# CityU-AIM-Group/MultiModal-learning

Measured on AMD Instinct MI355X. Metric: ROI-tiles/sec (teacher+student distill step), higher is better.
Workload: dtype bf16; 1 GPU; BASELINE configs[1]: teacher+student distill step, bf16, batch 64 per GPU, 512x512 tiles, 320-d omic, CRD P=300/K=700->P2=20/K2=512, n_data=1024, GK-Refine on, Adam+EMA, dropout 0.1; tiles_per_gpu=64, tile=512, global_batch=64, parallelism=single, launch=one captured HIP graph per step, input_pipeline=inputs resident in HBM when the timed region starts

## Files before the change

### multimodal-learning_amd/csrc/conv_wgrad.hip

```cpp
#include "ph_common.h"
#include "ph_kernels.h"
#include "tap_common.h"

namespace {

__device__ __forceinline__ int sw_piece(int pix, int piece) { return piece ^ (((pix >> 1) & 1) << 1); }

template <typename T, int S, int TH, int KS>
struct WgCfg {
  static constexpr bool SPLIT = is_f32<T>::value;
  static constexpr bool HPM = is_hp<T>::value;
  static constexpr int TW = 16, BM = TH * TW;
  static constexpr int HPH = (TH - 1) * S + KS, HPW = (TW - 1) * S + KS, HP = HPH * HPW;
  static constexpr int HPP = (HP + 7) / 8 * 8;
  static constexpr int D_BYTES = BM * 128, X_BYTES = HPP * 128;
  static constexpr int NP = SPLIT ? PH_NPLANES : 1;
  static constexpr int LDS_BYTES = SPLIT ? (D_BYTES + X_BYTES) * NP : 2 * (D_BYTES + X_BYTES);
  static constexpr int NT = KS * KS;
};

template <typename T>
__device__ __forceinline__ void stage_row(const T* src, bool ok, unsigned char* base, int plane_bytes, int off) {
  if constexpr (!is_f32<T>::value) {
    u32x4 v = {0u, 0u, 0u, 0u};
    if (ok) v = *reinterpret_cast<const u32x4*>(src);
    *reinterpret_cast<u32x4*>(base + off) = v;
  } else {
    float v[8];
#pragma unroll
    for (int q = 0; q < 8; ++q) v[q] = 0.f;
    if (ok) load8(src, v);
    bf16x8 p0, p1, p2;
#pragma unroll
    for (int q = 0; q < 8; ++q) { bf16 a, b, c; split3_bf16(v[q], a, b, c); p0[q] = a; p1[q] = b; p2[q] = c; }
    *reinterpret_cast<bf16x8*>(base + off) = p0;
    *reinterpret_cast<bf16x8*>(base + plane_bytes + off) = p1;
    *reinterpret_cast<bf16x8*>(base + 2 * plane_bytes + off) = p2;
  }
}

__device__ __forceinline__ bf16x8 tr_pair(const unsigned char* base, int off0, int off1) {
  typedef __attribute__((address_space(3))) s16x4 lds_s16x4;
  s16x4 a = __builtin_amdgcn_ds_read_tr16_b64_v4i16((lds_s16x4*)(base + off0));
  s16x4 b = __builtin_amdgcn_ds_read_tr16_b64_v4i16((lds_s16x4*)(base + off1));
  union { s16x4 s[2]; bf16x8 v; } u;
  u.s[0] = a; u.s[1] = b;
  return u.v;
}

template <typename T, int S, int TH, int KS>
__global__ __launch_bounds__(256) void wgrad_kernel(PhWgrad p) {
  using C = WgCfg<T, S, TH, KS>;
  constexpr bool SPLIT = C::SPLIT, HPM = C::HPM;
  constexpr int TW = C::TW, BM = C::BM, HPW = C::HPW, HP = C::HP, NT = C::NT, NP = C::NP;
  typedef typename std::conditional<HPM, f16, T>::type TI;
  constexpr int EW = HPM ? 2 : 1;
  extern __shared__ __attribute__((aligned(16))) unsigned char smem[];
  unsigned char* ldsD = smem;
  unsigned char* ldsX = smem + C::D_BYTES * NP;

  const int tid = threadIdx.x, lane = tid & 63;
  const int wave = __builtin_amdgcn_readfirstlane(tid >> 6);
  const int cf = wave >> 1, kf = wave & 1;
  const int cin_blocks = p.Cin >> 6;
  const int co0 = (blockIdx.x / cin_blocks) << 6, ci0 = (blockIdx.x % cin_blocks) << 6;
  const int chunk = blockIdx.y;
  const int tiles_w = (p.OW + TW - 1) / TW, tiles_h = (p.OH + TH - 1) / TH;
  const int tiles_img = tiles_w * tiles_h, ntiles = tiles_img * p.B;
  const int t_begin = chunk * p.tiles_per_chunk;
  const int t_end = min(ntiles, t_begin + p.tiles_per_chunk);
  const TI* X = reinterpret_cast<const TI*>(p.x);
  const TI* DY = reinterpret_cast<const TI*>(p.dy);
  const long xpix = (p.x_pix_stride ? p.x_pix_stride : p.Cin) * EW;
  const long xrow = (p.x_row_stride ? p.x_row_stride : (long)p.IW * p.Cin) * EW;
  const long ximg = (p.x_img_stride ? p.x_img_stride : (long)p.IH * p.IW * p.Cin) * EW;
  const long dpix = (long)p.Cout * EW;

  f32x16 acc[NT];
#pragma unroll
  for (int t = 0; t < NT; ++t)
#pragma unroll
    for (int q = 0; q < 16; ++q) acc[t][q] = 0.f;

  const int q4 = (lane & 15) >> 2, p4 = lane & 3, colhalf = (lane >> 4) & 1, khalf = lane >> 5;
  const int pieceA = cf * 2 + colhalf, pieceB = kf * 2 + colhalf;

  auto compute = [&](const unsigned char* dD, const unsigned char* dX) {
#pragma unroll 2
    for (int kk = 0; kk < BM / 16; ++kk) {
      const int t0 = kk * 16 + 8 * khalf + q4, t1 = t0 + 4;
      const int offA0 = t0 * 128 + sw_piece(t0, pieceA) * 32 + p4 * 8;
      const int offA1 = t1 * 128 + sw_piece(t1, pieceA) * 32 + p4 * 8;
      bf16x8 a[NP];
#ifdef PH_ABL_WG_NOLDS
#pragma unroll
      for (int pl = 0; pl < NP; ++pl) { bf16x8 z; asm volatile("" : "=v"(z)); a[pl] = z; }
#else
#pragma unroll
      for (int pl = 0; pl < NP; ++pl)
        if (pl < 2 || p.prod6) a[pl] = tr_pair(dD + pl * C::D_BYTES, offA0, offA1);
#endif
      const int hb0 = ((t0 >> 4) * S) * HPW + (t0 & 15) * S;
      const int hb1 = ((t1 >> 4) * S) * HPW + (t1 & 15) * S;
#pragma unroll
      for (int t = 0; t < NT; ++t) {
        const int toff = (t / KS) * HPW + (t % KS);
        const int h0 = hb0 + toff, h1 = hb1 + toff;
        const int offB0 = h0 * 128 + sw_piece(h0, pieceB) * 32 + p4 * 8;
        const int offB1 = h1 * 128 + sw_piece(h1, pieceB) * 32 + p4 * 8;
        bf16x8 bq[NP];
#ifdef PH_ABL_WG_NOLDS
#pragma unroll
        for (int pl = 0; pl < NP; ++pl) { bf16x8 z; asm volatile("" : "=v"(z) : "v"(offB0 + offB1)); bq[pl] = z; }
#else
#pragma unroll
        for (int pl = 0; pl < NP; ++pl)
          if (pl < 2 || p.prod6) bq[pl] = tr_pair(dX + pl * C::X_BYTES, offB0, offB1);
#endif
        if constexpr (SPLIT) {
#define PH_MM(PI, PJ) acc[t] = __builtin_amdgcn_mfma_f32_32x32x16_bf16(a[PI], bq[PJ], acc[t], 0, 0, 0);
          if (p.prod6) { PH_SPLIT_PAIRS_LO(PH_MM) }
          PH_SPLIT_PAIRS_HI(PH_MM)
#undef PH_MM
        } else if constexpr (HPM) {
          acc[t] = __builtin_amdgcn_mfma_f32_32x32x16_f16(__builtin_bit_cast(f16x8, a[0]), __builtin_bit_cast(f16x8, bq[0]), acc[t], 0, 0, 0);
        } else {
          acc[t] = __builtin_amdgcn_mfma_f32_32x32x16_bf16(a[0], bq[0], acc[t], 0, 0, 0);
        }
      }
    }
  };

  constexpr bool PIPE = !SPLIT && S == 1 && KS == 3 && (BM / 16 == TH);
  constexpr int PBUF = C::D_BYTES + C::X_BYTES;
  const int u_lane = 8 * khalf + q4;
  const int baseA = u_lane * 128 + ((pieceA ^ (((u_lane >> 1) & 1) << 1)) << 5) + p4 * 8;
  const int baseB = u_lane * 128 + (pieceB << 5) + p4 * 8;
  const int bE0 = baseB ^ (((u_lane >> 1) & 1) << 6), bE1 = bE0 ^ 64;
  const int bO0 = baseB ^ ((((u_lane >> 1) ^ u_lane) & 1) << 6), bO1 = bO0 ^ 64;
  if constexpr (PIPE) {
#pragma unroll
    for (int t = 0; t < NT; ++t) asm volatile("" : "+a"(acc[t]));
  }
  auto compute_p = [&](const int boff) __attribute__((always_inline)) {
    if constexpr (PIPE) {
      const unsigned char* dD = smem + boff;
      const unsigned char* dX = dD + C::D_BYTES;
      constexpr int NI = (BM / 16) * 9, LA = 3;
      bf16x8 af[2], bfr[4];
      auto ldA = [&](const int kk) { return tr_pair(dD, baseA + kk * 2048, baseA + 512 + kk * 2048); };
      auto ldB = [&](const int i) {
        const int kk = i / 9, t = i % 9;
        const int toff = (t / 3) * HPW + (t % 3);
        const int flip = ((kk & 1) ^ ((toff >> 1) & 1)) & 1;
        const int base = (toff & 1) ? (flip ? bO1 : bO0) : (flip ? bE1 : bE0);
        const int imm = (kk * HPW + toff) * 128;
        return tr_pair(dX, base + imm, base + imm + 512);
      };
      af[0] = ldA(0);
#pragma unroll
      for (int i = 0; i < LA; ++i) bfr[i] = ldB(i);
#pragma unroll
      for (int i = 0; i < NI; ++i) {
        const int kk = i / 9, t = i % 9;
        if (i + LA < NI) bfr[(i + LA) & 3] = ldB(i + LA);
        if (t == 4 && kk + 1 < BM / 16) af[(kk + 1) & 1] = ldA(kk + 1);
        if constexpr (HPM) asm volatile("v_mfma_f32_32x32x16_f16 %0, %1, %2, %0" : "+a"(acc[t]) : "v"(af[kk & 1]), "v"(bfr[i & 3]));
        else asm volatile("v_mfma_f32_32x32x16_bf16 %0, %1, %2, %0" : "+a"(acc[t]) : "v"(af[kk & 1]), "v"(bfr[i & 3]));
        __builtin_amdgcn_sched_barrier(0);
      }
    }
  };

  if constexpr (SPLIT) {
    for (int tt = t_begin; tt < t_end; ++tt) {
      const int b = tt / tiles_img, ti = tt - b * tiles_img;
      const int r0 = (ti / tiles_w) * TH, c0 = (ti % tiles_w) * TW;
      __syncthreads();
      for (int i = tid; i < BM * 8; i += 256) {
        const int pix = i >> 3, ch = i & 7;
        const int r = r0 + (pix >> 4), c = c0 + (pix & 15);
        const bool ok = r < p.OH && c < p.OW;
        const int off = pix * 128 + sw_piece(pix, ch >> 1) * 32 + (ch & 1) * 16;
        stage_row<T>(DY + (((size_t)b * p.OH + r) * p.OW + c) * p.Cout + co0 + ch * 8, ok, ldsD, C::D_BYTES, off);
      }
      const int iy_base = r0 * S - p.pad, ix_base = c0 * S - p.pad;
      for (int i = tid; i < HP * 8; i += 256) {
        const int pix = i >> 3, ch = i & 7;
        const int hr = pix / HPW, hc = pix - hr * HPW;
        const int iy = iy_base + hr, ix = ix_base + hc;
        const bool ok = iy >= 0 && iy < p.IH && ix >= 0 && ix < p.IW;
        const int off = pix * 128 + sw_piece(pix, ch >> 1) * 32 + (ch & 1) * 16;
        stage_row<T>(X + (size_t)b * ximg + (size_t)iy * xrow + (size_t)ix * xpix + ci0 + ch * 8, ok, ldsX, C::X_BYTES, off);
      }
      __syncthreads();
      compute(ldsD, ldsX);
    }
  } else {
    const unsigned lds0 = (unsigned)(size_t)(lds_uchar*)smem;
    constexpr int BUF = C::D_BYTES + C::X_BYTES;
    const unsigned char* zero = reinterpret_cast<const unsigned char*>(p.zeros);
    const int nt = t_end > t_begin ? t_end - t_begin : 0;
    const bool hi1 = HPM && p.hp_hi_only;
    const int nitems = (HPM && !hi1) ? 3 * nt : nt;
    const int dblk = HPM ? (co0 >> 6) * 128 : co0, xblk = HPM ? (ci0 >> 6) * 128 : ci0;
    auto issue = [&](int item, int buf) {
      int pass = 0, tt = t_begin + item;
      if constexpr (HPM) { if (!hi1) { pass = item / nt; tt = t_begin + (item - pass * nt); } else pass = 2; }
      const int dpl = (HPM && pass == 1) ? 64 : 0, xpl = (HPM && pass == 0) ? 64 : 0;
      const int b = tt / tiles_img, ti = tt - b * tiles_img;
      const int r0 = (ti / tiles_w) * TH, c0 = (ti % tiles_w) * TW;
      unsigned char* dD = smem + buf * BUF;
      unsigned char* dX = dD + C::D_BYTES;
      for (int i0 = wave * 64; i0 < BM * 8; i0 += 256) {
        const int i = i0 + lane, pix = i >> 3, pos = i & 7;
        const int ch = sw_piece(pix, pos >> 1) * 2 + (pos & 1);
        const int r = r0 + (pix >> 4), c = c0 + (pix & 15);
        const bool ok = r < p.OH && c < p.OW;
        const void* src = ok ? (const void*)(DY + (((size_t)b * p.OH + r) * p.OW + c) * dpix + dblk + dpl + ch * 8)
                             : (const void*)zero;
        lds_dma16(src, __builtin_amdgcn_readfirstlane(lds0 + (unsigned)(dD - smem) + i0 * 16));
      }
      const int iy_base = r0 * S - p.pad, ix_base = c0 * S - p.pad;
      for (int i0 = wave * 64; i0 < C::HPP * 8; i0 += 256) {
        const int i = i0 + lane, pix = i >> 3, pos = i & 7;
        const int ch = sw_piece(pix, pos >> 1) * 2 + (pos & 1);
        const int hr = pix / HPW, hc = pix - hr * HPW;
        const int iy = iy_base + hr, ix = ix_base + hc;
        const bool ok = pix < HP && iy >= 0 && iy < p.IH && ix >= 0 && ix < p.IW;
        const void* src = ok ? (const void*)(X + (size_t)b * ximg + (size_t)iy * xrow + (size_t)ix * xpix + xblk + xpl + ch * 8)
                             : (const void*)zero;
        lds_dma16(src, __builtin_amdgcn_readfirstlane(lds0 + (unsigned)(dX - smem) + i0 * 16));
      }
    };
    if (nitems > 0) issue(0, 0);
    asm volatile("s_waitcnt vmcnt(0)" ::: "memory");
    __syncthreads();
    int buf = 0;
    for (int it = 0; it < nitems; ++it) {
#ifndef PH_ABL_WG_NODMA
      if (it + 1 < nitems) issue(it + 1, buf ^ 1);
#endif
      if constexpr (HPM) {
        if (!hi1 && it == 2 * nt) {
#pragma unroll
          for (int t = 0; t < NT; ++t)
#pragma unroll
            for (int q = 0; q < 16; ++q) {
              if constexpr (PIPE) {
                float tmp_;
                asm volatile("v_accvgpr_read_b32 %1, %0\n\ts_nop 4\n\tv_mul_f32 %1, %2, %1\n\ts_nop 4\n\tv_accvgpr_write_b32 %0, %1\n\ts_nop 4"
                             : "+a"(acc[t][q]), "=&v"(tmp_) : "v"(PH_HP_LO_INV));
              } else {
                acc[t][q] *= PH_HP_LO_INV;
              }
            }
        }
      }
      if constexpr (PIPE) compute_p(buf * PBUF);
      else compute(smem + buf * BUF, smem + buf * BUF + C::D_BYTES);
      asm volatile("s_waitcnt vmcnt(0)" ::: "memory");
      __syncthreads();
      buf ^= 1;
    }
  }
  float* slab = p.slab + (size_t)chunk * NT * p.Cout * p.Cin;
#pragma unroll
  for (int t = 0; t < NT; ++t)
#pragma unroll
    for (int q = 0; q < 16; ++q) {
      const int row = co0 + cf * 32 + (q & 3) + 8 * (q >> 2) + 4 * khalf;
      const int col = ci0 + kf * 32 + (lane & 31);
#ifdef PH_ABL_WG_NOSLAB
      asm volatile("" ::"v"(acc[t][q]), "v"(row + col));
#else
      if constexpr (PIPE) {
        float* dst = slab + ((size_t)t * p.Cout + row) * p.Cin + col;
        asm volatile("global_store_dword %0, %1, off" : : "v"(dst), "a"(acc[t][q]) : "memory");
      } else {
        slab[((size_t)t * p.Cout + row) * p.Cin + col] = acc[t][q];
      }
#endif
      if (PIPE && q == 15) __builtin_amdgcn_sched_barrier(0);
    }
}

template <typename T, int S, int TH, int KS>
int launch_wg(const PhWgrad& p, hipStream_t st) {
  using C = WgCfg<T, S, TH, KS>;
  auto kern = wgrad_kernel<T, S, TH, KS>;
  static bool attr_done = false;
  if (!attr_done) {
    if (hipFuncSetAttribute(reinterpret_cast<const void*>(kern), hipFuncAttributeMaxDynamicSharedMemorySize,
                            C::LDS_BYTES) != hipSuccess)
      return PH_ELAUNCH;
    attr_done = true;
  }
  dim3 grid((p.Cout / 64) * (p.Cin / 64), p.nchunks);
  void* tok = nullptr;
  if (ph_prof_on())
    ph_prof_begin2(PH_CLS_WGRAD, 2.0 * p.B * p.OH * p.OW * (double)p.Cout * p.KS * p.KS * p.Cin,
                   ((double)p.B * p.IH * p.IW * p.Cin + (double)p.B * p.OH * p.OW * p.Cout) * sizeof(T) +
                       (double)p.nchunks * p.KS * p.KS * p.Cout * p.Cin * 4.0, st, &tok);
  hipLaunchKernelGGL(kern, grid, dim3(256), C::LDS_BYTES, st, p);
  ph_prof_end(tok, st);
  PH_LAUNCH_CHECK();
  return PH_OK;
}

template <typename T>
int launch_wg_T(const PhWgrad& p, hipStream_t st) {
  if (p.S == 1 && p.KS == 3) return launch_wg<T, 1, 8, 3>(p, st);
  if (p.S == 2 && p.KS == 3) return launch_wg<T, 2, 4, 3>(p, st);
  if (p.S == 2 && p.KS == 1) return launch_wg<T, 2, 4, 1>(p, st);
  if (p.S == 1 && p.KS == 1) return launch_wg<T, 1, 8, 1>(p, st);
  return PH_EINVAL;
}

__global__ __launch_bounds__(256) void wgrad_reduce_kernel(const float* __restrict__ slab, float* __restrict__ dw,
                                                           int nchunks, int NT, int Cout, int Cin,
                                                           const float* __restrict__ unscale) {
  const size_t n = (size_t)NT * Cout * Cin;
  const int e = threadIdx.x & 63, cl = threadIdx.x >> 6;
  const size_t i = (size_t)blockIdx.x * 64 + e;
  float s0 = 0.f, s1 = 0.f, s2 = 0.f, s3 = 0.f;
  if (i < n) {
    int c = cl;
    for (; c + 12 < nchunks; c += 16) {
      s0 += slab[(size_t)c * n + i];
      s1 += slab[(size_t)(c + 4) * n + i];
      s2 += slab[(size_t)(c + 8) * n + i];
      s3 += slab[(size_t)(c + 12) * n + i];
    }
    for (; c < nchunks; c += 4) s0 += slab[(size_t)c * n + i];
  }
  __shared__ float sh[4][64];
  sh[cl][e] = (s0 + s1) + (s2 + s3);
  __syncthreads();
  if (cl == 0 && i < n) {
    float s = (sh[0][e] + sh[1][e]) + (sh[2][e] + sh[3][e]);
    if (unscale) s *= unscale[1];
    const int ci = i % Cin;
    const int co = (i / Cin) % Cout;
    const int t = i / ((size_t)Cin * Cout);
    dw[((size_t)co * Cin + ci) * NT + t] = s;
  }
}

__global__ void pack_w_kernel(const float* __restrict__ w, bf16* __restrict__ planes, int O, int I, int NT,
                              int dgrad) {
  const size_t n = (size_t)NT * O * I;
  const size_t i = (size_t)blockIdx.x * blockDim.x + threadIdx.x;
  if (i >= n) return;
  int t, o, ii;
  if (!dgrad) { ii = i % I; o = (i / I) % O; t = i / ((size_t)I * O); }
  else        { o = i % O; ii = (i / O) % I; t = i / ((size_t)I * O); }
  const float v = w[((size_t)o * I + ii) * NT + t];
  bf16 a, b, c;
  split3_bf16(v, a, b, c);
  planes[i] = a; planes[n + i] = b; planes[2 * n + i] = c;
}

__global__ void pack_w_stem_kernel(const float* __restrict__ w, bf16* __restrict__ planes) {
  const int i = blockIdx.x * blockDim.x + threadIdx.x;
  if (i >= 7 * 64 * 32) return;
  const int k = i & 31, co = (i >> 5) & 63, kh = i >> 11;
  const int kw = k >> 2, ch = k & 3;
  float v = 0.f;
  if (kw < 7 && ch < 3) v = w[((co * 3 + ch) * 7 + kh) * 7 + kw];
  bf16 a, b, c;
  split3_bf16(v, a, b, c);
  planes[i] = a; planes[7 * 64 * 32 + i] = b; planes[2 * 7 * 64 * 32 + i] = c;
}

__global__ void pack_all_kernel(PhPackAll t, bf16* __restrict__ packed, int nplanes) {
  const size_t i = (size_t)blockIdx.x * blockDim.x + threadIdx.x;
  if (i >= t.total) return;
  int u = 0;
#pragma unroll 1
  while (u + 1 < t.n && i >= t.start[u + 1]) ++u;
  const size_t e = i - t.start[u];
  const int O = t.O[u], I = t.I[u], NT = t.NT[u];
  const size_t n = (size_t)NT * O * I;
  const int ii = e % I, o = (e / I) % O, tp = e / ((size_t)I * O);
  const float v = t.w[u][((size_t)o * I + ii) * NT + tp];
  bf16 a, b, c;
  split3_bf16(v, a, b, c);
  const size_t fdst = t.dst_fwd[u] + e;
  const size_t ddst = t.dst_dg[u] + ((size_t)tp * I + ii) * O + o;
  packed[fdst] = a; packed[ddst] = a;
  if (nplanes == 3) {
    packed[fdst + n] = b; packed[fdst + 2 * n] = c;
    packed[ddst + n] = b; packed[ddst + 2 * n] = c;
  }
}

struct PackTiles { int tstart[21]; };
__device__ __forceinline__ size_t frag64_index(int r, int k) {
  return (size_t)(((k >> 5) * 4 + (r & 3)) * 512 + ((((k >> 3) & 3) << 4) + (r >> 2)) * 8 + (k & 7));
}
template <int NP>
__global__ __launch_bounds__(256) void pack_all_tiled_kernel(PhPackAll t, PackTiles pt, bf16* __restrict__ packed) {
  __shared__ bf16 sh[NP][32][32 * 9 + 2];
  int u = 0;
#pragma unroll 1
  while (u + 1 < t.n && (int)blockIdx.x >= pt.tstart[u + 1]) ++u;
  const int O = t.O[u], I = t.I[u], NT = t.NT[u];
  const int tile = (int)blockIdx.x - pt.tstart[u];
  const int itiles = I >> 5;
  const int o0 = (tile / itiles) << 5, i0 = (tile % itiles) << 5;
  const size_t n = (size_t)NT * O * I;
  const int run = 32 * NT;
  for (int idx = threadIdx.x; idx < 32 * run; idx += 256) {
    const int o = idx / run, r = idx - o * run;
    const float v = t.w[u][((size_t)(o0 + o) * I + i0) * NT + r];
    if constexpr (NP == 1) {
      sh[0][o][r] = (bf16)v;
    } else {
      bf16 a, b, c;
      split3_bf16(v, a, b, c);
      sh[0][o][r] = a; sh[1][o][r] = b; sh[2][o][r] = c;
    }
  }
  __syncthreads();
  for (int idx = threadIdx.x; idx < 32 * run; idx += 256) {
    const int x = idx & 31, y = (idx >> 5) & 31, tp = idx >> 10;
    const size_t fdst = t.dst_fwd[u] + ((size_t)tp * O + o0 + y) * I + i0 + x;
    const size_t ddst = t.dst_dg[u] + ((size_t)tp * I + i0 + y) * O + o0 + x;
#pragma unroll
    for (int pl = 0; pl < NP; ++pl) {
      packed[fdst + pl * n] = sh[pl][y][x * NT + tp];
      packed[ddst + pl * n] = sh[pl][x][y * NT + tp];
    }
    if constexpr (NP == 1) {
      if (NT == 9 && O == 2 * I) {
        const int o = o0 + y, i = i0 + x;
        packed[t.dst_fwd[u] + n + (size_t)tp * O * I + (size_t)((o >> 6) * (I >> 6) + (i >> 6)) * 4096 + frag64_index(o & 63, i & 63)] = sh[0][y][x * NT + tp];
      }
      if (NT == 9 && O == I && I >= 128) {
        const int o = o0 + y, i = i0 + x;
        packed[t.dst_fwd[u] + n + (size_t)tp * O * I + (size_t)((o >> 6) * (I >> 6) + (i >> 6)) * 4096 + frag64_index(o & 63, i & 63)] = sh[0][y][x * NT + tp];
        const int r = i0 + y, k = o0 + x;
        packed[t.dst_dg[u] + n + (size_t)tp * I * O + (size_t)((r >> 6) * (O >> 6) + (k >> 6)) * 4096 + frag64_index(r & 63, k & 63)] = sh[0][x][y * NT + tp];
      }
    }
  }
}

__device__ __forceinline__ size_t hp_k(int k) { return (size_t)(k >> 6) * 192 + (k & 63); }
__device__ __forceinline__ void hp_w3(float v, f16& b0, f16& b1, f16& b2) {
  hp_split(v, b2, b1);
  b0 = (f16)((float)b2 * PH_HP_LO);
}
__device__ __forceinline__ size_t ph5_frag_index(int r, int k) { return frag64_index(r, k); }
template <bool ONE>
__global__ __launch_bounds__(256) void pack_all_tiled_hp_kernel(PhPackAll t, PackTiles pt, f16* __restrict__ packed, int dgrad_only) {
  __shared__ float sh[32][32 * 9 + 1];
  int u = 0;
#pragma unroll 1
  while (u + 1 < t.n && (int)blockIdx.x >= pt.tstart[u + 1]) ++u;
  const int O = t.O[u], I = t.I[u], NT = t.NT[u];
  const int ffwd = t.frag[u] & 3, fdg = (t.frag[u] >> 2) & 3;
  const int tile = (int)blockIdx.x - pt.tstart[u];
  const int itiles = I >> 5;
  const int o0 = (tile / itiles) << 5, i0 = (tile % itiles) << 5;
  const int run = 32 * NT;
  for (int idx = threadIdx.x; idx < 32 * run; idx += 256) {
    const int o = idx / run, r = idx - o * run;
    sh[o][r] = t.w[u][((size_t)(o0 + o) * I + i0) * NT + r];
  }
  __syncthreads();
  for (int idx = threadIdx.x; idx < 32 * run; idx += 256) {
    const int x = idx & 31, y = (idx >> 5) & 31, tp = idx >> 10;
    f16 b0, b1, b2;
    if (!ONE || dgrad_only == 0) {
      hp_w3(sh[y][x * NT + tp], b0, b1, b2);
      if (ffwd == PH_WFRAG_TAP5) {
        f16* d = packed + t.dst_fwd[u] + (size_t)tp * 12288 + ph5_frag_index(o0 + y, i0 + x);
        d[0] = b0; d[4096] = b1; d[8192] = b2;
      } else if (ffwd == PH_WFRAG_TAP6) {
        const int o = o0 + y, i = i0 + x;
        f16* d = packed + t.dst_fwd[u] + (size_t)tp * O * 3 * I + (size_t)(((o >> 6) * (I >> 6) + (i >> 6)) * 3) * 4096 + ph5_frag_index(o & 63, i & 63);
        d[0] = b0; d[4096] = b1; d[8192] = b2;
      } else {
        f16* d = packed + t.dst_fwd[u] + ((size_t)tp * O + o0 + y) * (3 * (size_t)I) + hp_k(i0 + x);
        d[0] = b0; d[64] = b1; d[128] = b2;
      }
    }
    if (!ONE || dgrad_only == 1) {
      hp_w3(sh[x][y * NT + tp], b0, b1, b2);
      if (fdg == PH_WFRAG_TAP5) {
        f16* d = packed + t.dst_dg[u] + (size_t)tp * 12288 + ph5_frag_index(i0 + y, o0 + x);
        d[0] = b0; d[4096] = b1; d[8192] = b2;
      } else {
        f16* d = packed + t.dst_dg[u] + ((size_t)tp * I + i0 + y) * (3 * (size_t)O) + hp_k(o0 + x);
        d[0] = b0; d[64] = b1; d[128] = b2;
      }
    }
  }
}

__global__ void pack_w_stem_hp_kernel(const float* __restrict__ w, f16* __restrict__ packed) {
  const int i = blockIdx.x * blockDim.x + threadIdx.x;
  if (i >= 7 * 64 * 32) return;
  const int k = i & 31, co = (i >> 5) & 63, kh = i >> 11;
  const int kw = k >> 2, ch = k & 3;
  float v = 0.f;
  if (kw < 7 && ch < 3) v = w[((co * 3 + ch) * 7 + kh) * 7 + kw];
  f16 b0, b1, b2;
  hp_w3(v, b0, b1, b2);
  packed[i] = b0; packed[7 * 64 * 32 + i] = b1; packed[2 * 7 * 64 * 32 + i] = b2;
}

}

int ph_pack_w_stem_hp_launch(const float* w, void* packed, hipStream_t st) {
  hipLaunchKernelGGL(pack_w_stem_hp_kernel, dim3((7 * 64 * 32 + 255) / 256), dim3(256), 0, st, w, (f16*)packed);
  PH_LAUNCH_CHECK();
  return PH_OK;
}

int ph_pack_w_hp_launch(const float* w, void* packed, int O, int I, int KS, int dgrad, int wfrag, hipStream_t st) {
  if ((O & 31) || (I & 31) || (KS != 1 && KS != 3)) return PH_EINVAL;
  if (wfrag == PH_WFRAG_TAP5 && !(O == 64 && I == 64 && KS == 3)) return PH_EINVAL;
  if (wfrag == PH_WFRAG_TAP6 && !(O == 2 * I && KS == 3 && !dgrad)) return PH_EINVAL;
  if (wfrag < 0 || wfrag > PH_WFRAG_TAP6) return PH_EINVAL;
  PhPackAll t{};
  t.n = 1; t.w[0] = w; t.O[0] = O; t.I[0] = I; t.NT[0] = KS * KS; t.dst_fwd[0] = 0; t.dst_dg[0] = 0;
  t.frag[0] = dgrad ? wfrag << 2 : wfrag;
  t.start[0] = 0; t.start[1] = t.total = (size_t)KS * KS * O * I;
  PackTiles pt;
  pt.tstart[0] = 0; pt.tstart[1] = (O >> 5) * (I >> 5);
  hipLaunchKernelGGL(pack_all_tiled_hp_kernel<true>, dim3(pt.tstart[1]), dim3(256), 0, st, t, pt, (f16*)packed, dgrad ? 1 : 0);
  PH_LAUNCH_CHECK();
  return PH_OK;
}

int ph_pack_all_launch(const PhPackAll* t, void* packed, int nplanes, hipStream_t st) {
  bool tiled = t->n <= 20;
  PackTiles pt;
  pt.tstart[0] = 0;
  for (int u = 0; u < t->n && tiled; ++u) {
    if ((t->O[u] & 31) || (t->I[u] & 31) || t->NT[u] > 9) tiled = false;
    pt.tstart[u + 1] = pt.tstart[u] + (t->O[u] >> 5) * (t->I[u] >> 5);
  }
  if (nplanes == -3) {
    if (!tiled) return PH_EINVAL;
    for (int u = 0; u < t->n; ++u) {
      const int ff = t->frag[u] & 3, fd = (t->frag[u] >> 2) & 3;
      if ((ff == PH_WFRAG_TAP5 || fd == PH_WFRAG_TAP5) && !(t->O[u] == 64 && t->I[u] == 64 && t->NT[u] == 9)) return PH_EINVAL;
      if (ff == PH_WFRAG_TAP6 && !(t->O[u] == 2 * t->I[u] && t->NT[u] == 9)) return PH_EINVAL;
      if (ff == 3 || fd == 3 || fd == PH_WFRAG_TAP6) return PH_EINVAL;
    }
    hipLaunchKernelGGL(pack_all_tiled_hp_kernel<false>, dim3(pt.tstart[t->n]), dim3(256), 0, st, *t, pt, (f16*)packed, 0);
  } else if (tiled && nplanes == 1)
    hipLaunchKernelGGL(pack_all_tiled_kernel<1>, dim3(pt.tstart[t->n]), dim3(256), 0, st, *t, pt, (bf16*)packed);
  else if (tiled && nplanes == 3)
    hipLaunchKernelGGL(pack_all_tiled_kernel<3>, dim3(pt.tstart[t->n]), dim3(256), 0, st, *t, pt, (bf16*)packed);
  else
    hipLaunchKernelGGL(pack_all_kernel, dim3((unsigned)((t->total + 255) / 256)), dim3(256), 0, st, *t, (bf16*)packed,
                       nplanes);
  PH_LAUNCH_CHECK();
  return PH_OK;
}

int ph_wgrad_tile_h(int S) { return S == 1 ? 8 : 4; }

int ph_wgrad_launch(const PhWgrad* p, int prec, hipStream_t st) {
  if (p->Cin % 64 || p->Cout % 64 || p->nchunks < 1) return PH_EINVAL;
  if (prec == PH_PREC_BF16) { ph_dispatch_note(PH_DK_WGRAD_BF16); return launch_wg_T<bf16>(*p, st); }
  if (prec == PH_PREC_FP16X3 || prec == PH_PREC_FP16X1) {
    PhWgrad q = *p;
    q.hp_hi_only = prec == PH_PREC_FP16X1;
    ph_dispatch_note(PH_DK_WGRAD_HP16);
    return launch_wg_T<hp16>(q, st);
  }
  if (PH_IS_SPLIT_PREC(prec)) {
    PhWgrad q = *p;
    q.prod6 = prec == PH_PREC_BF16X6;
    ph_dispatch_note(PH_DK_WGRAD_F32);
    return launch_wg_T<float>(q, st);
  }
  return PH_EINVAL;
}

int ph_wgrad_reduce_launch(const float* slab, float* dw, int nchunks, int KS, int Cout, int Cin, const float* unscale,
                           hipStream_t st) {
  const size_t n = (size_t)KS * KS * Cout * Cin;
  hipLaunchKernelGGL(wgrad_reduce_kernel, dim3((unsigned)((n + 63) / 64)), dim3(256), 0, st, slab, dw, nchunks,
                     KS * KS, Cout, Cin, unscale);
  PH_LAUNCH_CHECK();
  return PH_OK;
}

int ph_pack_w_fwd_launch(const float* w, void* planes, int O, int I, int KS, hipStream_t st) {
  const size_t n = (size_t)KS * KS * O * I;
  hipLaunchKernelGGL(pack_w_kernel, dim3((unsigned)((n + 255) / 256)), dim3(256), 0, st, w, (bf16*)planes, O, I,
                     KS * KS, 0);
  PH_LAUNCH_CHECK();
  return PH_OK;
}
int ph_pack_w_dgrad_launch(const float* w, void* planes, int O, int I, int KS, hipStream_t st) {
  const size_t n = (size_t)KS * KS * O * I;
  hipLaunchKernelGGL(pack_w_kernel, dim3((unsigned)((n + 255) / 256)), dim3(256), 0, st, w, (bf16*)planes, O, I,
                     KS * KS, 1);
  PH_LAUNCH_CHECK();
  return PH_OK;
}
int ph_pack_w_stem_launch(const float* w, void* planes, hipStream_t st) {
  hipLaunchKernelGGL(pack_w_stem_kernel, dim3((7 * 64 * 32 + 255) / 256), dim3(256), 0, st, w, (bf16*)planes);
  PH_LAUNCH_CHECK();
  return PH_OK;
}
```

Measured before the change: 6354 tiles/s.

## Add lean wgrad loop with precomputed DMA offsets and reordered MFMA reuse

Adds a LEAN variant of the weight-gradient kernel, gated by a PH_WG_LEAN switch. It precomputes per-lane LDS-DMA offsets and validity bitmasks once per block and walks tiles incrementally, instead of recomputing addresses and bounds for every item. Its compute loop reorders the MFMA stream so each staged halo row fragment serves all three kh taps. DMA issues for the next item are interleaved into the MFMA stream. The cost is more kernel variants and register state. Whether it runs depends on the switch default and on a 32-bit offset fit check.

Result: faster. 6479 tiles/s (median of 6 runs) (+2.0%).

```diff
diff --git a/multimodal-learning_amd/csrc/conv_wgrad.hip b/multimodal-learning_amd/csrc/conv_wgrad.hip
--- a/multimodal-learning_amd/csrc/conv_wgrad.hip
+++ b/multimodal-learning_amd/csrc/conv_wgrad.hip
@@ -1,6 +1,8 @@
 #include "ph_common.h"
 #include "ph_kernels.h"
 #include "tap_common.h"
+
+PH_SWITCH(wg_lean, "PH_WG_LEAN")
 
 namespace {
 
@@ -17,6 +19,7 @@
   static constexpr int NP = SPLIT ? PH_NPLANES : 1;
   static constexpr int LDS_BYTES = SPLIT ? (D_BYTES + X_BYTES) * NP : 2 * (D_BYTES + X_BYTES);
   static constexpr int NT = KS * KS;
+  static constexpr int NDP = BM * 8 / 256, NHP = (HPP * 8 + 255) / 256, NPIECES = NDP + NHP;
 };
 
 template <typename T>
@@ -48,11 +51,12 @@
   return u.v;
 }
 
-template <typename T, int S, int TH, int KS>
+template <typename T, int S, int TH, int KS, bool LEAN>
 __global__ __launch_bounds__(256) void wgrad_kernel(PhWgrad p) {
   using C = WgCfg<T, S, TH, KS>;
   constexpr bool SPLIT = C::SPLIT, HPM = C::HPM;
-  constexpr int TW = C::TW, BM = C::BM, HPW = C::HPW, HP = C::HP, NT = C::NT, NP = C::NP;
+  constexpr int TW = C::TW, BM = C::BM, HPH = C::HPH, HPW = C::HPW, HP = C::HP, NT = C::NT, NP = C::NP;
+  static_assert(!(LEAN && SPLIT), "the lean loop is a perf-mode (LDS-DMA) loop");
   typedef typename std::conditional<HPM, f16, T>::type TI;
   constexpr int EW = HPM ? 2 : 1;
   extern __shared__ __attribute__((aligned(16))) unsigned char smem[];
@@ -171,6 +175,43 @@
       }
     }
   };
+  auto compute_l = [&](const int boff, auto dma) __attribute__((always_inline)) {
+    if constexpr (PIPE && LEAN) {
+      const unsigned char* dD = smem + boff;
+      const unsigned char* dX = dD + C::D_BYTES;
+      constexpr int NF = (TH + 2) * 3, LF = 3, DMA_FIRST = 0, DMA_STEP = 1;
+      bf16x8 af[4], bfr[4];
+      auto ldA = [&](const int kk) { return tr_pair(dD, baseA + kk * 2048, baseA + 512 + kk * 2048); };
+      auto ldB = [&](const int j) {
+        const int hoff = (j / 3) * HPW + (j % 3);
+        const int flip = (hoff >> 1) & 1;
+        const int base = (hoff & 1) ? (flip ? bO1 : bO0) : (flip ? bE1 : bE0);
+        return tr_pair(dX, base + hoff * 128, base + hoff * 128 + 512);
+      };
+      af[0] = ldA(0);
+#pragma unroll
+      for (int j = 0; j < LF; ++j) bfr[j] = ldB(j);
+      int m = 0;
+#pragma unroll
+      for (int j = 0; j < NF; ++j) {
+        const int h = j / 3, kw = j % 3;
+        if (j + LF < NF) bfr[(j + LF) & 3] = ldB(j + LF);
+        if (kw == 1 && h + 1 < TH) af[(h + 1) & 3] = ldA(h + 1);
+#pragma unroll
+        for (int kh = 0; kh < 3; ++kh) {
+          const int kk = h - kh;
+          if (kk >= 0 && kk < TH) {
+            if constexpr (HPM) asm volatile("v_mfma_f32_32x32x16_f16 %0, %1, %2, %0" : "+a"(acc[kh * 3 + kw]) : "v"(af[kk & 3]), "v"(bfr[j & 3]));
+            else asm volatile("v_mfma_f32_32x32x16_bf16 %0, %1, %2, %0" : "+a"(acc[kh * 3 + kw]) : "v"(af[kk & 3]), "v"(bfr[j & 3]));
+            __builtin_amdgcn_sched_barrier(0);
+            if (m >= DMA_FIRST && (m - DMA_FIRST) % DMA_STEP == 0) { dma((m - DMA_FIRST) / DMA_STEP); __builtin_amdgcn_sched_barrier(0); }
+            ++m;
+          }
+        }
+      }
+      static_assert((TH * 9 - 1 - DMA_FIRST) / DMA_STEP + 1 >= C::NPIECES, "every piece of the next item has a slot in the MFMA stream");
+    }
+  };
 
   if constexpr (SPLIT) {
     for (int tt = t_begin; tt < t_end; ++tt) {
@@ -196,7 +237,7 @@
       __syncthreads();
       compute(ldsD, ldsX);
     }
-  } else {
+  } else if constexpr (!LEAN) {
     const unsigned lds0 = (unsigned)(size_t)(lds_uchar*)smem;
     constexpr int BUF = C::D_BYTES + C::X_BYTES;
     const unsigned char* zero = reinterpret_cast<const unsigned char*>(p.zeros);
@@ -263,6 +304,144 @@
       __syncthreads();
       buf ^= 1;
     }
+  } else {
+    static_assert(BM * 8 % 256 == 0, "whole dz pieces per wave");
+    constexpr int NDP = C::NDP, NHP = C::NHP, NPC = C::NPIECES;
+    constexpr bool H_TAIL = (C::HPP * 8) % 256 != 0;
+    typedef typename std::conditional<(HPH + HPW < 32), unsigned, unsigned long long>::type hmask_t;
+    const unsigned lds0 = (unsigned)(size_t)(lds_uchar*)smem;
+    constexpr int BUF = C::D_BYTES + C::X_BYTES;
+    const unsigned char* zero = reinterpret_cast<const unsigned char*>(p.zeros);
+    const int nt = t_end > t_begin ? t_end - t_begin : 0;
+    const bool hi1 = HPM && p.hp_hi_only;
+    const int nitems = (HPM && !hi1) ? 3 * nt : nt;
+    const int dblk = HPM ? (co0 >> 6) * 128 : co0, xblk = HPM ? (ci0 >> 6) * 128 : ci0;
+    unsigned d_off[NDP], d_pos[NDP], h_off[NHP];
+    hmask_t h_pos[NHP];
+#pragma unroll
+    for (int k = 0; k < NDP; ++k) {
+      const int i = wave * 64 + 256 * k + lane, pix = i >> 3, pos = i & 7;
+      const int ch = sw_piece(pix, pos >> 1) * 2 + (pos & 1);
+      d_off[k] = (unsigned)((((long)(pix >> 4) * p.OW + (pix & 15)) * dpix + ch * 8) * 2);
+      d_pos[k] = (1u << (pix >> 4)) | (1u << (TH + (pix & 15)));
+    }
+#pragma unroll
+    for (int k = 0; k < NHP; ++k) {
+      const int i = wave * 64 + 256 * k + lane, pix = i >> 3, pos = i & 7;
+      const int ch = sw_piece(pix, pos >> 1) * 2 + (pos & 1);
+      const int hr = pix / HPW, hc = pix - hr * HPW;
+      const bool in = pix < HP;
+      h_off[k] = in ? (unsigned)(((long)hr * xrow + (long)hc * xpix + ch * 8) * 2) : 0u;
+      h_pos[k] = in ? ((hmask_t)1 << hr) | ((hmask_t)1 << (HPH + hc)) : (hmask_t)1 << (HPH + HPW);
+    }
+    typedef const unsigned char* bptr;
+    const int b_s = t_begin / tiles_img, ti_s = t_begin - b_s * tiles_img;
+    const int trow_s = ti_s / tiles_w, tcol_s = ti_s - trow_s * tiles_w;
+    auto d_at = [&](int b, int trow, int tcol) {
+      return reinterpret_cast<bptr>(DY) + ((((long)b * p.OH + trow * TH) * p.OW + tcol * TW) * dpix + dblk) * 2;
+    };
+    auto x_at = [&](int b, int trow, int tcol) {
+      return reinterpret_cast<bptr>(X) + ((long)b * ximg + (long)(trow * TH * S - p.pad) * xrow + (long)(tcol * TW * S - p.pad) * xpix + xblk) * 2;
+    };
+    const long d_col = (long)TW * dpix * 2, d_row = (long)TH * p.OW * dpix * 2, d_img = (long)p.OH * p.OW * dpix * 2;
+    const long x_col = (long)TW * S * xpix * 2, x_row = (long)TH * S * xrow * 2, x_img = ximg * 2;
+    int crow = trow_s, ccol = tcol_s, cpass = hi1 ? 2 : 0, cleft = nt;
+    bptr od, od_r, od_i, ox, ox_r, ox_i;
+    unsigned dv_r, dv_c;
+    hmask_t hv_r, hv_c;
+    auto span = [](int lo, int hi) -> hmask_t {
+      return hi > lo ? (((hmask_t)1 << hi) - 1) & ~(((hmask_t)1 << lo) - 1) : (hmask_t)0;
+    };
+    auto row_words = [&]() {
+      const int r0 = crow * TH, iy_base = r0 * S - p.pad;
+      dv_r = (unsigned)span(0, min(TH, p.OH - r0));
+      hv_r = span(max(0, -iy_base), min(HPH, p.IH - iy_base));
+    };
+    auto col_words = [&]() {
+      const int c0 = ccol * TW, ix_base = c0 * S - p.pad;
+      dv_c = (unsigned)span(0, min(TW, p.OW - c0)) << TH;
+      hv_c = span(max(0, -ix_base), min(HPW, p.IW - ix_base)) << HPH;
+    };
+    auto to_start = [&]() {
+      crow = trow_s; ccol = tcol_s;
+      od = d_at(b_s, trow_s, tcol_s); od_r = d_at(b_s, trow_s, 0); od_i = d_at(b_s, 0, 0);
+      ox = x_at(b_s, trow_s, tcol_s); ox_r = x_at(b_s, trow_s, 0); ox_i = x_at(b_s, 0, 0);
+      row_words();
+    };
+    to_start();
+    col_words();
+    bptr nx_d = zero, nx_x = zero;
+    unsigned nx_dv = 0;
+    hmask_t nx_hv = 0;
+    auto next_item = [&](const bool have) {
+      nx_d = od + ((HPM && cpass == 1) ? 128 : 0);
+      nx_x = ox + ((HPM && cpass == 0) ? 128 : 0);
+      nx_dv = have ? dv_r | dv_c : 0u;
+      nx_hv = have ? hv_r | hv_c : (hmask_t)0;
+      ++ccol; od += d_col; ox += x_col;
+      if (ccol == tiles_w) {
+        ccol = 0; ++crow; od_r += d_row; ox_r += x_row;
+        if (crow == tiles_h) { crow = 0; od_i += d_img; ox_i += x_img; od_r = od_i; ox_r = ox_i; }
+        od = od_r; ox = ox_r;
+        row_words();
+      }
+      if constexpr (HPM) { if (--cleft == 0) { cleft = nt; ++cpass; to_start(); } }
+      col_words();
+    };
+    unsigned ldst = lds0 + wave * 1024;
+    auto dma = [&](const int k) __attribute__((always_inline)) {
+#ifndef PH_ABL_WG_NODMA
+      if (k < NDP) {
+        const unsigned char* src = (d_pos[k] & nx_dv) == d_pos[k] ? nx_d + d_off[k] : zero;
+        lds_dma16(src, ldst + k * 4096);
+      } else if (k < NPC) {
+        const int e = k - NDP;
+        if (H_TAIL && e == NHP - 1 && wave * 64 + 256 * e >= C::HPP * 8) return;
+        const unsigned char* src = (h_pos[e] & nx_hv) == h_pos[e] ? nx_x + h_off[e] : zero;
+        lds_dma16(src, ldst + C::D_BYTES + e * 4096);
+      }
+#endif
+    };
+    if (nitems > 0) {
+      next_item(true);
+#pragma unroll
+      for (int k = 0; k < NPC; ++k) dma(k);
+    }
+    asm volatile("s_waitcnt vmcnt(0)" ::: "memory");
+    __syncthreads();
+    int buf = 0;
+    for (int it = 0; it < nitems; ++it) {
+      next_item(it + 1 < nitems);
+      ldst = lds0 + (buf ^ 1) * BUF + wave * 1024;
+      if constexpr (HPM) {
+        if (!hi1 && it == 2 * nt) {
+#pragma unroll
+          for (int t = 0; t < NT; ++t)
+#pragma unroll
+            for (int q = 0; q < 16; ++q) {
+              if constexpr (PIPE) {
+                float tmp_;
+                asm volatile("v_accvgpr_read_b32 %1, %0\n\ts_nop 4\n\tv_mul_f32 %1, %2, %1\n\ts_nop 4\n\tv_accvgpr_write_b32 %0, %1\n\ts_nop 4"
+                             : "+a"(acc[t][q]), "=&v"(tmp_) : "v"(PH_HP_LO_INV));
+              } else {
+                acc[t][q] *= PH_HP_LO_INV;
+              }
+            }
+        }
+      }
+      if constexpr (PIPE) {
+        compute_l(buf * PBUF, dma);
+      } else {
+        if (it + 1 < nitems) {
+#pragma unroll
+          for (int k = 0; k < NPC; ++k) dma(k);
+        }
+        compute(smem + buf * BUF, smem + buf * BUF + C::D_BYTES);
+      }
+      asm volatile("s_waitcnt vmcnt(0)" ::: "memory");
+      __syncthreads();
+      buf ^= 1;
+    }
   }
   float* slab = p.slab + (size_t)chunk * NT * p.Cout * p.Cin;
 #pragma unroll
@@ -286,9 +465,20 @@
 }
 
 template <typename T, int S, int TH, int KS>
-int launch_wg(const PhWgrad& p, hipStream_t st) {
+bool wg_lean_fits(const PhWgrad& p) {
   using C = WgCfg<T, S, TH, KS>;
-  auto kern = wgrad_kernel<T, S, TH, KS>;
+  const long EW = C::HPM ? 2 : 1;
+  const long xpix = (p.x_pix_stride ? p.x_pix_stride : p.Cin) * EW;
+  const long xrow = (p.x_row_stride ? p.x_row_stride : (long)p.IW * p.Cin) * EW;
+  const long xmax = ((long)C::HPH * xrow + (long)C::HPW * xpix + 128) * 2;
+  const long dmax = (((long)TH * p.OW + C::TW) * p.Cout * EW + 128) * 2;
+  return xrow >= 0 && xpix >= 0 && xmax < (1L << 32) && dmax < (1L << 32);
+}
+
+template <typename T, int S, int TH, int KS, bool LEAN>
+int launch_wg_k(const PhWgrad& p, hipStream_t st) {
+  using C = WgCfg<T, S, TH, KS>;
+  auto kern = wgrad_kernel<T, S, TH, KS, LEAN>;
   static bool attr_done = false;
   if (!attr_done) {
     if (hipFuncSetAttribute(reinterpret_cast<const void*>(kern), hipFuncAttributeMaxDynamicSharedMemorySize,
@@ -306,6 +496,14 @@
   ph_prof_end(tok, st);
   PH_LAUNCH_CHECK();
   return PH_OK;
+}
+
+template <typename T, int S, int TH, int KS>
+int launch_wg(const PhWgrad& p, hipStream_t st) {
+  if constexpr (!is_f32<T>::value) {
+    if (ph_wg_lean_switch(-1) && wg_lean_fits<T, S, TH, KS>(p)) return launch_wg_k<T, S, TH, KS, true>(p, st);
+  }
+  return launch_wg_k<T, S, TH, KS, false>(p, st);
 }
 
 template <typename T>
```
